# cnmoro/MiniVectorDB

Hardware: AMD Instinct MI355X
Metric: queries/sec + p50 latency, brute-force IP kNN, 10M×512 fp32, k=10 (higher is better)
Workload: dtype f32; 1 GPU; 10000000 x 512 fp32 corpus (10000000 rows resident per GPU), IP, k=10, nq=1 per step; rows_per_gpu=10000000, dim=512, k=10, nq=1, parallelism=row-sharded x1

## Files before the change

include/mvdb.h:

```cpp
#ifndef MVDB_H
#define MVDB_H

#include <stdint.h>

#ifdef __cplusplus
extern "C" {
#endif

#define MVDB_METRIC_IP 0
#define MVDB_METRIC_L2 1

#define MVDB_OK 0
#define MVDB_ERR_ARG 1
#define MVDB_ERR_HIP 2
#define MVDB_ERR_NODEVICE 3
#define MVDB_ERR_OOM 4

typedef struct mvdb_index mvdb_index;
typedef struct mvdb_encoder mvdb_encoder;


const char* mvdb_last_error(void);

int mvdb_abi_version(void);
// ... 14 lines not shown
int64_t mvdb_index_ntotal(const mvdb_index* idx);
int mvdb_index_dim(const mvdb_index* idx);
int mvdb_index_device(const mvdb_index* idx);

int64_t mvdb_index_shadow_rows(const mvdb_index* idx);

int64_t mvdb_index_code8_rows(const mvdb_index* idx);

int mvdb_index_code8_counters(const mvdb_index* idx, long long* fallbacks, long long* last_candidates, long long* calls);

int mvdb_code8_margin(int d, float qnorm, float qstep, float row_norm_bound, float* alpha, float* beta);

int mvdb_code8_pack(int d, const int8_t* codes, uint8_t* high, uint8_t* low);
int mvdb_code8_unpack(int d, const uint8_t* high, const uint8_t* low, int8_t* codes);

int mvdb_code8_front_pack(int d, const int8_t* codes, uint8_t* image);
int mvdb_code8_front_unpack(int d, const uint8_t* image, int8_t* codes);

int mvdb_code8_front_geometry(int d, int64_t n, int device, int* rows_per_batch, int* waves);

int mvdb_index_code8_front_counters(const mvdb_index* idx, long long* survivors, long long* calls, long long* suspensions, int* held);

int mvdb_index_code8_read_row(const mvdb_index* idx, int64_t row, uint8_t* high, uint8_t* low, uint8_t* front);

int mvdb_code8_scan_geometry(int d, int64_t n, int device, int* rows_per_batch, int* waves);

int mvdb_index_code8_refined(const mvdb_index* idx, long long* rows);

int mvdb_index_reserve(mvdb_index* idx, int64_t n);

int mvdb_index_add(mvdb_index* idx, const float* x_host, int64_t n, int normalize);

int mvdb_index_add_device(mvdb_index* idx, const float* x_dev, int64_t n, int normalize);

int mvdb_index_add_synthetic(mvdb_index* idx, int64_t n, uint64_t seed, int64_t first_row,
                             int normalize);

int mvdb_index_get_rows(const mvdb_index* idx, int64_t row0, int64_t n, float* out_host);

int mvdb_index_remove_rows(mvdb_index* idx, const int64_t* rows_host, int64_t m);

int mvdb_index_set_rows(mvdb_index* idx, const int64_t* rows_host, const float* x_host, int64_t m, int normalize);

int mvdb_index_set_rows_device(mvdb_index* idx, const int64_t* rows_host, const float* x_dev , int64_t m,
                               int normalize);

// ... 205 lines not shown
```

minivectordb_amd/_native.py:

```python
import ctypes
import os

import numpy as np

_HERE = os.path.dirname(os.path.abspath(__file__))
LIB_PATH = os.path.join(_HERE, "lib", "libmvdb.so")
LIB_PATH = os.environ.get("MVDB_LIBMVDB", LIB_PATH)

METRIC_IP = 0
METRIC_L2 = 1

ERR_ARG = 1
ERR_HIP = 2
ERR_NODEVICE = 3
ERR_OOM = 4

_lib = None

c_f32p = ctypes.POINTER(ctypes.c_float)
c_i64p = ctypes.POINTER(ctypes.c_int64)
c_i32p = ctypes.POINTER(ctypes.c_int32)
c_vp = ctypes.c_void_p


# ... 14 lines not shown

PROTOTYPES = {
    "mvdb_last_error": (ctypes.c_char_p, []),
    "mvdb_abi_version": (ctypes.c_int, []),
    "mvdb_device_count": (ctypes.c_int, [ctypes.POINTER(ctypes.c_int)]),
    "mvdb_index_create": (ctypes.c_int, [ctypes.c_int, ctypes.c_int, ctypes.c_int, ctypes.POINTER(c_vp)]),
    "mvdb_index_free": (ctypes.c_int, [c_vp]),
    "mvdb_index_reload_env": (ctypes.c_int, [c_vp]),
    "mvdb_index_set_option": (ctypes.c_int, [c_vp, ctypes.c_char_p, ctypes.c_longlong]),
    "mvdb_index_reset": (ctypes.c_int, [c_vp]),
    "mvdb_index_ntotal": (ctypes.c_int64, [c_vp]),
    "mvdb_index_shadow_rows": (ctypes.c_int64, [c_vp]),
    "mvdb_index_code8_rows": (ctypes.c_int64, [c_vp]),
    "mvdb_index_code8_counters": (ctypes.c_int, [c_vp, c_vp, c_vp, c_vp]),
    "mvdb_code8_margin": (ctypes.c_int, [ctypes.c_int, ctypes.c_float, ctypes.c_float, ctypes.c_float, c_vp, c_vp]),
    "mvdb_code8_pack": (ctypes.c_int, [ctypes.c_int, c_vp, c_vp, c_vp]),
    "mvdb_code8_unpack": (ctypes.c_int, [ctypes.c_int, c_vp, c_vp, c_vp]),
    "mvdb_index_code8_refined": (ctypes.c_int, [c_vp, c_vp]),
    "mvdb_code8_front_pack": (ctypes.c_int, [ctypes.c_int, c_vp, c_vp]),
    "mvdb_code8_front_unpack": (ctypes.c_int, [ctypes.c_int, c_vp, c_vp]),
    "mvdb_code8_front_geometry": (ctypes.c_int, [ctypes.c_int, ctypes.c_int64, ctypes.c_int, c_vp, c_vp]),
    "mvdb_index_code8_front_counters": (ctypes.c_int, [c_vp, c_vp, c_vp, c_vp, c_vp]),
    "mvdb_index_code8_read_row": (ctypes.c_int, [c_vp, ctypes.c_int64, c_vp, c_vp, c_vp]),
    "mvdb_code8_scan_geometry": (ctypes.c_int, [ctypes.c_int, ctypes.c_int64, ctypes.c_int, c_vp, c_vp]),
    "mvdb_index_dim": (ctypes.c_int, [c_vp]),
    "mvdb_index_device": (ctypes.c_int, [c_vp]),
    "mvdb_index_reserve": (ctypes.c_int, [c_vp, ctypes.c_int64]),
    "mvdb_index_add": (ctypes.c_int, [c_vp, c_vp, ctypes.c_int64, ctypes.c_int]),
    "mvdb_index_add_device": (ctypes.c_int, [c_vp, c_vp, ctypes.c_int64, ctypes.c_int]),
    "mvdb_index_add_synthetic": (ctypes.c_int, [c_vp, ctypes.c_int64, ctypes.c_uint64, ctypes.c_int64, ctypes.c_int]),
    "mvdb_index_get_rows": (ctypes.c_int, [c_vp, ctypes.c_int64, ctypes.c_int64, c_vp]),
    "mvdb_index_remove_rows": (ctypes.c_int, [c_vp, c_vp, ctypes.c_int64]),
    "mvdb_index_set_rows": (ctypes.c_int, [c_vp, c_vp, c_vp, ctypes.c_int64, ctypes.c_int]),
    "mvdb_index_set_rows_device": (ctypes.c_int, [c_vp, c_vp, c_vp, ctypes.c_int64, ctypes.c_int]),
    "mvdb_index_search": (ctypes.c_int, [c_vp, c_vp, ctypes.c_int, ctypes.c_int, ctypes.c_int, c_vp, c_vp]),
    "mvdb_index_search_device": (ctypes.c_int, [c_vp, c_vp, ctypes.c_int, ctypes.c_int, ctypes.c_int,
                                                ctypes.c_int64, c_vp, c_vp, c_vp]),
    "mvdb_index_search_subset": (ctypes.c_int, [c_vp, c_vp, ctypes.c_int, ctypes.c_int, ctypes.c_int, c_vp,
                                                ctypes.c_int64, c_vp, c_vp]),
    "mvdb_index_search_subset_device": (ctypes.c_int, [c_vp, c_vp, ctypes.c_int, ctypes.c_int, ctypes.c_int, c_vp,
                                                       ctypes.c_int64, ctypes.c_int, ctypes.c_int64, c_vp, c_vp, c_vp]),
    "mvdb_index_search_masked": (ctypes.c_int, [c_vp, c_vp, ctypes.c_int, ctypes.c_int, ctypes.c_int, c_vp, ctypes.c_int,
                                                c_vp, c_vp]),
    "mvdb_index_search_masked_device": (ctypes.c_int, [c_vp, c_vp, ctypes.c_int, ctypes.c_int, ctypes.c_int, c_vp,
                                                       ctypes.c_int, ctypes.c_int64, c_vp, c_vp, c_vp]),
    "mvdb_rowset_create": (ctypes.c_int, [c_vp, c_vp, ctypes.c_int64, ctypes.c_int, ctypes.POINTER(c_vp)]),
# ... 979 lines not shown

def code8_front_pack(codes):
    codes = np.ascontiguousarray(codes, dtype=np.int8)
    d = codes.shape[0]
    image = np.empty(max(d // 8 * 5, 1), np.uint8)
    check(lib().mvdb_code8_front_pack(int(d), codes.ctypes.data, image.ctypes.data))
    return image


def code8_front_unpack(image):
    image = np.ascontiguousarray(image, dtype=np.uint8)
    d = image.shape[0] // 5 * 8
    codes = np.empty(max(d, 1), np.int8)
    check(lib().mvdb_code8_front_unpack(int(d), image.ctypes.data, codes.ctypes.data))
    return codes


def code8_front_geometry(d, n, device=0):
    rb, waves = ctypes.c_int(0), ctypes.c_int(0)
    check(lib().mvdb_code8_front_geometry(int(d), int(n), int(device), ctypes.byref(rb), ctypes.byref(waves)))
    return int(rb.value), int(waves.value)


def code8_scan_geometry(d, n, device=0):
    rb, waves = ctypes.c_int(0), ctypes.c_int(0)
    check(lib().mvdb_code8_scan_geometry(int(d), int(n), int(device), ctypes.byref(rb), ctypes.byref(waves)))
    return int(rb.value), int(waves.value)
```

minivectordb_amd/csrc/code8_scan.hpp:

```cpp
#pragma once
#include "scan_kernels.hpp"

namespace mvdb {

typedef int i32x4 __attribute__((ext_vector_type(4)));

struct Code8Margin {
    float alpha, beta;
};
__host__ __device__ inline Code8Margin code8_margin(int d, float qnorm, float qstep, float row_norm_bound) {
    const double u = 5.9604644775390625e-08;
    const double qn = (double)qnorm, B = (double)row_norm_bound;
    const double dq = (double)qstep * sqrt((double)d) * 0.5 * 1.001 + qn * 4.0 * u;
    const double kap = 8.0 * u;
    const double gam = (d + 8) * u / (1.0 - (d + 8) * u);
    const double eta = 2.0 * (d + 16) * u;
    const double up = 1.0 + 9.5367431640625e-07;
    Code8Margin m;
    m.alpha = (float)((qn + dq) * (1.0 + kap) * up);
    m.beta = (float)(B * (dq + kap * (qn + dq) + (gam * (1.0 + eta) + eta) * qn) * up + 1e-30);
    return m;
}
__host__ __device__ inline int code8_qmax(int d) { return d <= 512 ? 32512 : 16256; }

// ... 27 lines not shown
#pragma unroll
    for (int i = 0; i < 4; ++i) c[i] |= lo[i];
}
inline void code8_pack_row(int d, const int8_t* codes, uint8_t* high, uint8_t* low) {
    for (int t = 0; t < d / 16; ++t) {
        uint32_t c[4], h[3], l;
        memcpy(c, codes + 16 * t, 16);
        code8_pack_chunk(c, h, l);
        memcpy(high + 12 * t, h, 12);
        memcpy(low + 4 * t, &l, 4);
    }
}
inline void code8_unpack_row(int d, const uint8_t* high, const uint8_t* low, int8_t* codes) {
    for (int t = 0; t < d / 16; ++t) {
        uint32_t c[4], h[3], l;
        memcpy(h, high + 12 * t, 12);
        memcpy(&l, low + 4 * t, 4);
        code8_unpack_chunk(h, l, c);
        memcpy(codes + 16 * t, c, 16);
    }
}

constexpr uint32_t kCode8FrontMask = 0xF8F8F8F8u;
__host__ __device__ inline bool code8_front_dim(int d) { return d > 0 && d % 32 == 0 && d <= 2048; }
__host__ __device__ inline int code8_front_stride(int d) { return d / 8 * 5; }
__host__ __device__ inline int code8_front_lanes(int d) {
    int g = 1;
    while (g * 32 < d) g *= 2;
    return g;
}
__host__ __device__ inline int code8_front_tile_rows(int d) { return 64 / code8_front_lanes(d); }
__host__ __device__ inline size_t code8_front_bytes(int64_t cap, int d) {
    const int64_t R = code8_front_tile_rows(d);
    return (size_t)((cap + R - 1) / R * R) * (size_t)code8_front_stride(d);
}
__host__ __device__ inline size_t code8_front_wide_offset(int64_t row, int d) {
    const int64_t R = code8_front_tile_rows(d);
    return (size_t)(row / R * R) * (size_t)code8_front_stride(d) + (size_t)(row % R) * (size_t)(d / 2);
}
__host__ __device__ inline size_t code8_front_narrow_offset(int64_t row, int d) {
    const int64_t R = code8_front_tile_rows(d);
    return (size_t)(row / R * R) * (size_t)code8_front_stride(d) + (size_t)R * (size_t)(d / 2) + (size_t)(row % R) * (size_t)(d / 8);
}

__host__ __device__ inline void code8_front_pack_chunk(const uint32_t (&c)[8], uint32_t (&f)[5]) {
    f[0] = (c[0] & kCode8FrontMask) | ((c[5] >> 5) & 0x07070707u);
    f[1] = (c[1] & kCode8FrontMask) | ((c[5] >> 3) & 0x03030303u) | ((c[7] >> 2) & 0x04040404u);
    f[2] = (c[2] & kCode8FrontMask) | ((c[6] >> 5) & 0x07070707u);
    f[3] = (c[3] & kCode8FrontMask) | ((c[6] >> 3) & 0x03030303u) | ((c[7] >> 1) & 0x04040404u);
    f[4] = (c[4] & kCode8FrontMask) | ((c[7] >> 5) & 0x07070707u);
}
__host__ __device__ inline void code8_front_unpack_chunk(const uint32_t (&f)[5], uint32_t (&c)[8]) {
#pragma unroll
    for (int i = 0; i < 5; ++i) c[i] = f[i] & kCode8FrontMask;
    c[5] = ((f[0] & 0x07070707u) << 5) | ((f[1] & 0x03030303u) << 3);
    c[6] = ((f[2] & 0x07070707u) << 5) | ((f[3] & 0x03030303u) << 3);
    c[7] = ((f[4] & 0x07070707u) << 5) | ((f[1] & 0x04040404u) << 2) | ((f[3] & 0x04040404u) << 1);
}
inline void code8_front_pack_row(int d, const int8_t* codes, uint8_t* image) {
    for (int t = 0; t < d / 32; ++t) {
        uint32_t c[8], f[5];
        memcpy(c, codes + 32 * t, 32);
        code8_front_pack_chunk(c, f);
        memcpy(image + 16 * t, f, 16);
        memcpy(image + d / 2 + 4 * t, &f[4], 4);
// ... 49 lines not shown
                    float cf = rintf(v[j] / a);
                    cf = fminf(fmaxf(cf, -127.f), 127.f);
                    const float e = fmaf(-a, cf, v[j]);
                    r2 = fmaf(e, e, r2);
                    word |= ((uint32_t)(uint8_t)(int8_t)(int)cf) << (8 * j);
                }
            }
            uint32_t chunk[4], h[3], l;
#pragma unroll
            for (int j = 0; j < 4; ++j) chunk[j] = (uint32_t)__shfl((int)word, (lane & ~3) + j);
            code8_pack_chunk(chunk, h, l);
            const int part = lane & 3;
            if (part < 3)
                hdst[3 * (c >> 2) + part] = part == 0 ? h[0] : part == 1 ? h[1] : h[2];
            else
                ldst[c >> 2] = l;
            if (front) {
                uint32_t oct[8], f[5];
#pragma unroll
                for (int j = 0; j < 8; ++j) oct[j] = (uint32_t)__shfl((int)word, (lane & ~7) + j);
                code8_front_pack_chunk(oct, f);
                const int fpart = lane & 7;
                if (fpart < 4)
                    reinterpret_cast<uint32_t*>(front + code8_front_wide_offset(front_row0 + row, d))[4 * (c >> 3) + fpart] =
                        fpart == 0 ? f[0] : fpart == 1 ? f[1] : fpart == 2 ? f[2] : f[3];
                else if (fpart == 4)
                    reinterpret_cast<uint32_t*>(front + code8_front_narrow_offset(front_row0 + row, d))[c >> 3] = f[4];
            }
        }
#pragma unroll
        for (int m = 32; m >= 1; m >>= 1) r2 += __shfl_xor(r2, m);
        if (lane == 0) {
            float r;
            if (anybad)
                r = INFINITY;
            else if (tiny)
                r = fmaf(mx, sqrtf((float)d) * 1.01f, 1e-44f);
            else
                r = sqrtf(r2 + (float)d * 2e-38f) * 1.001f;
            if (!(r < INFINITY)) r = INFINITY;
            ar[row] = make_float2(a, r);
        }
    }
}

constexpr int kCode8QueryThreads = 256;
constexpr int kCode8MaxDim = 1024;

struct Code8QueryShared {
    float nr[kCode8QueryThreads];
// ... 212 lines not shown

template <int G, int U, int M = 1>
__device__ __forceinline__ int code8_reduce(int (&T)[U], int t) {
    if constexpr (M < U) {
        constexpr int H = U / (2 * M);
        const bool hi = (t & M) != 0;
#pragma unroll
        for (int j = 0; j < H; ++j) {
            const int send = hi ? T[j] : T[j + H];
            const int keep = hi ? T[j + H] : T[j];
            T[j] = keep + lane_xor<M>(send);
        }
        return code8_reduce<G, U, M * 2>(T, t);
    } else if constexpr (M < G) {
        T[0] += lane_xor<M>(T[0]);
        return code8_reduce<G, U, M * 2>(T, t);
    } else {
        return T[0];
    }
}

typedef int i32x3 __attribute__((ext_vector_type(3), aligned(4)));

template <int G, int U, bool MASKED, int GF = 0, int UF = 0>
__global__ __launch_bounds__(kScanThreads) void code8_scan_kernel(Code8ScanArgs a) {
    constexpr int RPI = kWave / G;
    constexpr int RB = RPI * U;
    constexpr bool FRONT = GF > 0;
    static_assert(U >= 2 && U <= 8 && (U & (U - 1)) == 0 && U <= G, "code8_reduce halves U down to one value inside a row group");
    static_assert(!FRONT || (UF >= 2 && UF <= 8 && (UF & (UF - 1)) == 0 && UF <= GF && kWave % GF == 0), "the same, for the front form");
    const int lane = threadIdx.x & (kWave - 1);
    const int wave = __builtin_amdgcn_readfirstlane(threadIdx.x >> 6);
    const int t = lane % G;
    const int g = lane / G;
    const bool valid = !MASKED || t * 16 < a.d;

    i32x4 qh = {0, 0, 0, 0}, ql = {0, 0, 0, 0};
    if (valid) {
        qh = *reinterpret_cast<const i32x4*>(a.qhi + t * 16);
        ql = *reinterpret_cast<const i32x4*>(a.qlo + t * 16);
    }
    const float qstep = a.par[0], alpha = a.par[1], beta = a.par[2];
    float floor = 0.f;

    int p3 = 0, n3 = 0;
#pragma unroll
    for (int j = 0; j < 4; ++j) {
#pragma unroll
        for (int b = 0; b < 4; ++b) {
            const int Q = ((qh[j] << (24 - 8 * b)) >> 24) * 256 + ((ql[j] << (24 - 8 * b)) >> 24);
            p3 += Q > 0 ? Q : 0;
            n3 += Q < 0 ? -Q : 0;
        }
// ... 110 lines not shown
            const int src = __ffsll((long long)pass) - 1;
            pass &= pass - 1;
            const uint32_t v = (uint32_t)__builtin_amdgcn_readlane((int)r, src);
            const int w = __builtin_amdgcn_readlane(t6, src);
            if (lane == ns1) {
                srow = v;
                st6 = w;
            }
            if (++ns1 == kWave) refine();
        }
    };

    const int64_t nwaves_total = (int64_t)gridDim.x * kScanWaves;
    const int64_t gw = (int64_t)blockIdx.x * kScanWaves + wave;
    __shared__ uint64_t sh[(kScanWaves - 1) * kWave];
    __shared__ float sfloor;

    if constexpr (FRONT) {
        constexpr int RPF = kWave / GF;
        constexpr int RBF = RPF * UF;
        const int tf = lane % GF;
        const int gf = lane / GF;
        const bool validf = !MASKED || tf * 32 < a.d;
        i32x4 fh[2] = {{0, 0, 0, 0}, {0, 0, 0, 0}}, fl[2] = {{0, 0, 0, 0}, {0, 0, 0, 0}};
        if (validf) {
#pragma unroll
            for (int i = 0; i < 2; ++i) {
                fh[i] = *reinterpret_cast<const i32x4*>(a.qhi + tf * 32 + 16 * i);
                fl[i] = *reinterpret_cast<const i32x4*>(a.qlo + tf * 32 + 16 * i);
            }
        }
        int uef = 0;
#pragma unroll
        for (int m = 1, h = UF / 2; m < UF; m <<= 1, h >>= 1) uef += (tf & m) ? h : 0;
        const int erowf = uef * RPF + gf;
        const uint64_t elanesf = __ballot(tf < UF);

        if (blockIdx.x == 0 && threadIdx.x == 0) {
            const unsigned int calls = atomicAdd(a.front_calls, 1u);
            const unsigned long long sum = atomicAdd(a.front_survivors, 0ull);
            if (a.front_msum) {
                *a.front_msum = sum;
                *a.front_mcalls = calls;
            }
        }

        auto scores0 = [&](const i32x4 (&xw)[UF], const int (&xn)[UF], int (&T)[UF]) {
#pragma unroll
            for (int u = 0; u < UF; ++u) {
                const uint32_t f[5] = {(uint32_t)xw[u].x, (uint32_t)xw[u].y, (uint32_t)xw[u].z, (uint32_t)xw[u].w, (uint32_t)xn[u]};
                uint32_t c[8];
                code8_front_unpack_chunk(f, c);
                int hi = 0, lo = 0;
#pragma unroll
                for (int j = 0; j < 8; ++j) {
                    hi = __builtin_amdgcn_sdot4((int)c[j], fh[j >> 2][j & 3], hi, false);
                    lo = __builtin_amdgcn_sdot4((int)c[j], fl[j >> 2][j & 3], lo, false);
                }
                T[u] = hi * 256 + lo;
            }
        };
        uint32_t s0row = 0;
        int ns0 = 0;
        unsigned long long nfront = 0;
        auto gather0 = [&]() __attribute__((always_inline)) {
            nfront += (unsigned long long)ns0;
            for (int base = 0; base < ns0; base += RB) {
                i32x3 x[U];
#pragma unroll
                for (int u = 0; u < U; ++u) {
                    int e = base + u * RPI + g;
                    e = e < ns0 - 1 ? e : ns0 - 1;
                    const uint32_t row = (uint32_t)__shfl((int)s0row, e);
                    const i32x3* src = reinterpret_cast<const i32x3*>(a.high + (int64_t)row * a.hstride + t * 12);
                    if (MASKED)
                        x[u] = valid ? *src : i32x3{0, 0, 0};
                    else
                        x[u] = *src;
                }
                const int e = base + erow;
// ... 6 lines not shown
            }
            ns0 = 0;
        };
        auto stage0 = [&](int t5, float2 sr, uint64_t mine, int64_t r) __attribute__((always_inline)) {
            const int tl = (t5 > INT_MIN + n7 ? t5 : INT_MIN + n7) - n7;
            const float su = ((float)(t5 + p7) * qstep) * sr.x;
            const float sl = ((float)tl * qstep) * sr.x;
            float m = fmaf(alpha, sr.y, beta);
            m = fmaf(fmaxf(fabsf(su), fabsf(sl)) + m, 2.4e-7f, m);
            const float ub = su + m;
            uint64_t pass = __ballot(!(ub < floor)) & mine;
            while (pass) {
                const int src = __ffsll((long long)pass) - 1;
                pass &= pass - 1;
                const uint32_t v = (uint32_t)__builtin_amdgcn_readlane((int)r, src);
                if (lane == ns0) s0row = v;
                if (++ns0 == kWave) gather0();
            }
        };

        const int nch = a.d / 32;
        const int64_t tile_bytes = (int64_t)RPF * code8_front_stride(a.d);
        const int64_t batch_bytes = (int64_t)UF * tile_bytes;
        const int wide_off = gf * 16 * nch + tf * 16;
        const int narrow_off = RPF * 16 * nch + gf * 4 * nch + tf * 4;
        const int64_t nfull = a.n / RBF;
        auto load0 = [&](i32x4 (&xw)[UF], int (&xn)[UF], float2& sr, int64_t b) {
            const uint8_t* base = a.front + b * batch_bytes;
#pragma unroll
            for (int u = 0; u < UF; ++u) {
                const i32x4* ws = reinterpret_cast<const i32x4*>(base + u * tile_bytes + wide_off);
                const int* ns = reinterpret_cast<const int*>(base + u * tile_bytes + narrow_off);
                if (MASKED) {
                    xw[u] = validf ? __builtin_nontemporal_load(ws) : i32x4{0, 0, 0, 0};
                    xn[u] = validf ? __builtin_nontemporal_load(ns) : 0;
                } else {
                    xw[u] = __builtin_nontemporal_load(ws);
                    xn[u] = __builtin_nontemporal_load(ns);
                }
            }
            sr = a.ar[b * RBF + erowf];
        };
        int64_t b = gw;
        const bool head = b < nfull;
        i32x4 xw0[UF];
        int xn0[UF];
        float2 sr0 = make_float2(0.f, 0.f);
        if (head) load0(xw0, xn0, sr0, b);
        floor = __uint_as_float((uint32_t)__builtin_amdgcn_readfirstlane(
            (int)__float_as_uint(code8_lists_floor(a.lists, a.nlists, a.k, sh, &sfloor, kScanWaves))));
        if (blockIdx.x == 0 && threadIdx.x == 0) *a.floor = floor;
        if (head) {
            int T[UF];
            scores0(xw0, xn0, T);
            stage0(code8_reduce<GF, UF>(T, tf), sr0, elanesf, b * RBF + erowf);
            b += nwaves_total;
        }
        for (; b < nfull; b += nwaves_total) {
            i32x4 xw[UF];
            int xn[UF];
            float2 sr;
            load0(xw, xn, sr, b);
            int T[UF];
            scores0(xw, xn, T);
            stage0(code8_reduce<GF, UF>(T, tf), sr, elanesf, b * RBF + erowf);
        }
        if (nfull * RBF < a.n && nfull % nwaves_total == gw) {
            const int64_t last = a.n - 1;
            const int64_t last_tile = last / RPF;
            i32x4 xw[UF];
            int xn[UF];
#pragma unroll
            for (int u = 0; u < UF; ++u) {
                int64_t tile = nfull * UF + u;
                tile = tile < last_tile ? tile : last_tile;
                const uint8_t* base = a.front + tile * tile_bytes;
                const i32x4* ws = reinterpret_cast<const i32x4*>(base + wide_off);
                const int* ns = reinterpret_cast<const int*>(base + narrow_off);
                if (MASKED) {
                    xw[u] = validf ? __builtin_nontemporal_load(ws) : i32x4{0, 0, 0, 0};
                    xn[u] = validf ? __builtin_nontemporal_load(ns) : 0;
                } else {
                    xw[u] = __builtin_nontemporal_load(ws);
                    xn[u] = __builtin_nontemporal_load(ns);
                }
            }
            const int64_t r = nfull * RBF + erowf;
            const float2 sr = a.ar[r < last ? r : last];
            int T[UF];
            scores0(xw, xn, T);
            stage0(code8_reduce<GF, UF>(T, tf), sr, __ballot(tf < UF && r < a.n), r);
        }
        if (ns0) gather0();
        if (ns1) refine();
        if (nfront && lane == 0) atomicAdd(a.front_survivors, nfront);
        if (nrefined && lane == 0) atomicAdd(a.survivors, nrefined);
        if (nst) flush();
        return;
    }

    const int64_t nfull = a.n / RB;
    const int64_t batch_bytes = (int64_t)RB * a.hstride;
    const int64_t group_bytes = (int64_t)RPI * a.hstride;
    const int lane_off = g * a.hstride + t * 12;

    auto load = [&](i32x3 (&x)[U], float2& sr, int64_t b) {
        const uint8_t* base = a.high + b * batch_bytes + lane_off;
#pragma unroll
// ... 386 lines not shown
```

minivectordb_amd/csrc/mvdb.hip:

```cpp
#include <algorithm>
#include <cmath>
#include <cstdlib>
#include <atomic>
#include <functional>
#include <map>
#include <tuple>
#include <vector>
#include <shared_mutex>

#include "common.hpp"
#include "index_state.hpp"
#include "scan_kernels.hpp"
#include "grouped_scan.hpp"
#include "range_scan.hpp"
#include "join_scan.hpp"
#include "mmr_select.hpp"
#include "distinct_select.hpp"
#include "maxsim_scan.hpp"
#include "assign_scan.hpp"
#include "code8_scan.hpp"
#include "scan_mfma_kernels.hpp"
#include "select_kernels.hpp"
#include "half_scan.hpp"
#include "util_kernels.hpp"
// ... 1820 lines not shown
    rows = idx->n + n_new;
    return 0;
}

bool code8_route_ok(const mvdb_index* idx, int nq, int k, const int64_t* rows_dev, const uint64_t* mask_dev, int64_t n) {
    if (nq != 1 || !idx->kn.code8_single_query || idx->kn.shadow_single_query) return false;
    if (idx->metric != MVDB_METRIC_IP || rows_dev || mask_dev || k > kMaxFusedK) return false;
    if (n != idx->n || n < kCode8MinRows || !code8_dim(idx->d) || idx->ld != idx->d) return false;
    if (!(idx->row_norm_bound > 0.f) || !(idx->row_norm_bound < 1.0e30f) || idx->code.failed) return false;
    return true;
}

template <int G_, int U_, bool MASKED_, int SCAN_U_, int SCAN_BLOCKS_, int FRONT_G_, int FRONT_U_, int FRONT_BLOCKS_, bool FRONT_DEFAULT_>
struct Code8Shape {
    static constexpr bool FRONT_DEFAULT = FRONT_DEFAULT_;
    static constexpr int G = G_, U = U_, SCAN_U = SCAN_U_, SCAN_BLOCKS = SCAN_BLOCKS_;
    static constexpr int FRONT_G = FRONT_G_, FRONT_U = FRONT_U_, FRONT_BLOCKS = FRONT_BLOCKS_;
    static constexpr bool MASKED = MASKED_;
};
template <typename Launch>
int with_code8_shape(int d, Launch launch) {
    switch (d) {
        case 384: return launch(Code8Shape<32, 8, true, 8, 4, 16, 8, 2, true>{});
        case 512: return launch(Code8Shape<32, 4, false, 8, 2, 16, 4, 2, true>{});
        case 1024: return launch(Code8Shape<64, 4, false, 8, 2, 32, 4, 2, false>{});
        default: return fail(MVDB_ERR_ARG, "internal: no int8 prefilter kernel for d = %d", d);
    }
}
template <typename Launch>
int with_code8_exact_shape(int d4, Launch launch) {
    return with_scan_shape(d4, [&](auto shape) {
        if constexpr (code8_shape(decltype(shape)::G, decltype(shape)::C)) return launch(shape);
        else return fail(MVDB_ERR_ARG, "internal: no int8 prefilter kernel for rows of %d 16-byte chunks", d4);
    });
}

bool code8_front_wanted(int option, int d) {
    if (option == 0 || !code8_dim(d) || !code8_front_dim(d)) return false;
    bool dflt = false;
    (void)with_code8_shape(d, [&](auto cs) {
        dflt = decltype(cs)::FRONT_DEFAULT;
        return 0;
    });
    return option >= 2 || dflt;
}

template <int G, int U, bool MASKED, int BLOCKS, int GF = 0, int UF = 0>
int code8_scan_blocks(int64_t n, int device) {
    void (*kern)(Code8ScanArgs) = code8_scan_kernel<G, U, MASKED, GF, UF>;
    int per_cu = std::min(cached_occupancy((const void*)kern, kScanThreads, 0, 4), BLOCKS);
    if (kn().scan_blocks_per_cu > 0) per_cu = kn().scan_blocks_per_cu;
    return scan_grid(n, GF > 0 ? (kWave / GF) * UF : (kWave / G) * U, per_cu, device);
}
template <int G, int U, bool MASKED, int BLOCKS, int GF = 0, int UF = 0>
int launch_code8_scan(const Code8ScanArgs& a, int device, hipStream_t stream) {
    void (*kern)(Code8ScanArgs) = code8_scan_kernel<G, U, MASKED, GF, UF>;
    const int nblocks = code8_scan_blocks<G, U, MASKED, BLOCKS, GF, UF>(a.n, device);
    if constexpr (GF > 0)
        return profiled_launch("ip_scan", stream, [&](hipEvent_t done) { launch_kernel(kern, dim3(nblocks), dim3(kScanThreads), 0, stream, done, a); },
                               "code8_scan_kernel<%d, %d, %s, %d, %d>", G, U, MASKED ? "true" : "false", GF, UF);
    else
        return profiled_launch("ip_scan", stream, [&](hipEvent_t done) { launch_kernel(kern, dim3(nblocks), dim3(kScanThreads), 0, stream, done, a); },
                               "code8_scan_kernel<%d, %d, %s>", G, U, MASKED ? "true" : "false");
}
constexpr double kCode8FrontShare = 0.12;
bool code8_front_serves(const mvdb_index* idx) {
    if (!idx->code.F5.p || !code8_front_wanted(idx->kn.code8_front_plane, idx->d)) return false;
    if (idx->kn.code8_front_plane >= 2) return idx->kn.code8_front_plane == 2;
    const volatile unsigned long long* sum = idx->c8_ctr.mirror<unsigned long long>();
    return !idx->c8_front.suspended_mean(sum ? sum + 2 : nullptr, idx->c8_ctr.mirror() ? idx->c8_ctr.mirror() + 6 : nullptr,
                                         kCode8FrontShare * (double)idx->n);
}

template <int G, int U, bool MASKED>
int launch_code8_seed(const Code8SeedArgs& a, int device, hipStream_t stream, int* nlists) {
    void (*kern)(Code8SeedArgs) = code8_seed_kernel<G, U, MASKED>;
    int threads = kn().code8_seed_threads;
    if (threads != 256 && threads != 512 && threads != 1024) threads = kCode8SeedThreads;
    constexpr int64_t nbatches = kCode8Seed / ((kWave / G) * U);
    const int64_t want = (nbatches + threads / kWave - 1) / (threads / kWave);
    int64_t blocks = kn().code8_seed_blocks > 0 ? kn().code8_seed_blocks : device_cus(device);
    blocks = std::max<int64_t>(1, std::min<int64_t>(std::min<int64_t>(blocks, want), scan_grid_upper_bound(device)));
    *nlists = (int)blocks;
    return profiled_launch("ip_scan_code8_seed", stream, [&](hipEvent_t done) { launch_kernel(kern, dim3((unsigned)blocks), dim3(threads), 0, stream, done, a); },
                           "code8_seed_kernel<%d, %d, %s>", G, U, MASKED ? "true" : "false");
}

template <int G, int C, int U, bool MASKED>
int launch_code8_rescore(const Code8RescoreArgs& a, int device, hipStream_t stream) {
    void (*kern)(Code8RescoreArgs) = code8_rescore_kernel<G, C, U, MASKED>;
    const int64_t want = (a.cap + a.rows_per_block - 1) / a.rows_per_block;
    const int64_t blocks = std::max<int64_t>(1, std::min<int64_t>(want, (int64_t)device_cus(device) * 4));
    return profiled_launch("ip_scan_code8_rescore", stream, [&](hipEvent_t done) { launch_kernel(kern, dim3((unsigned)blocks), dim3(kScanThreads), 0, stream, done, a); },
                           "code8_rescore_kernel<%d, %d, %d, %s>", G, C, U, MASKED ? "true" : "false");
// ... 56 lines not shown
    c.n = idx->n;
    c.d = d;
    c.hstride = code8_high_stride(d);
    c.qhi = qhi;
    c.qlo = qlo;
    c.par = par;
    c.lists = ws->cand.p;
    c.nlists = seed_lists;
    c.k = k;
    c.floor = floor;
    c.cand = cand;
    c.cap = cap;
    c.counter = counter;
    c.survivors = reinterpret_cast<unsigned long long*>(idx->c8_ctr.dev() + 2);
    c.front = idx->code.F5.p;
    c.front_survivors = reinterpret_cast<unsigned long long*>(idx->c8_ctr.dev() + 4);
    c.front_calls = idx->c8_ctr.dev() + 6;
    c.front_msum = idx->c8_ctr.mirror<unsigned long long>() + 2;
    c.front_mcalls = idx->c8_ctr.mirror() + 6;
    const bool front = code8_front_serves(idx);
    MVDB_TRY(with_code8_shape(d, [&](auto cs) {
        using K = decltype(cs);
        if (!front) return launch_code8_scan<K::G, K::SCAN_U, K::MASKED, K::SCAN_BLOCKS>(c, idx->device, s);
        const int fu = kn().code8_front_u == 4 || kn().code8_front_u == 8 ? kn().code8_front_u : K::FRONT_U;
        if (fu == 4) return launch_code8_scan<K::G, K::SCAN_U, K::MASKED, K::FRONT_BLOCKS, K::FRONT_G, 4>(c, idx->device, s);
        return launch_code8_scan<K::G, K::SCAN_U, K::MASKED, K::FRONT_BLOCKS, K::FRONT_G, 8>(c, idx->device, s);
    }));
    Code8RescoreArgs r;
    r.X = a0.X;
    r.ld = a0.ld;
    r.d4 = a0.d4;
    r.q = a0.q;
    r.normalize_q = a0.normalize_q;
    r.k = k;
    r.cand = cand;
    r.counter = counter;
    r.cap = cap;
    r.par = par;
    r.rows_per_block = kn().code8_rescore_rows > 0 ? kn().code8_rescore_rows : kCode8RescoreRows;
    r.lists = ws->cand.p;
    r.active = active;
    r.gate = gate;
    r.ctr_dev = idx->c8_ctr.dev();
    r.stats = idx->c8_ctr.mirror();
    MVDB_TRY(with_code8_exact_shape(a0.d4, [&](auto shape) {
        using S = decltype(shape);
        return launch_code8_rescore<S::G, S::C, rescore_u(S::G, S::C), false>(r, idx->device, s);
    }));
    ScanArgs a = a0;
// ... 319 lines not shown
        std::lock_guard<std::mutex> lk(idx->shadow_mu);
        *held = idx->code.F5.p ? 1 : 0;
    }
    if (!idx->c8_ctr.dev()) return 0;
    DeviceGuard dg(idx->device);
    unsigned int w[3] = {0, 0, 0};
    MVDB_HIP(hipMemcpy(w, idx->c8_ctr.dev() + 4, sizeof(w), hipMemcpyDeviceToHost));
    if (survivors) *survivors = (long long)((unsigned long long)w[0] | ((unsigned long long)w[1] << 32));
    if (calls) *calls = (long long)w[2];
    return 0;
}
int mvdb_index_code8_read_row(const mvdb_index* idx, int64_t row, uint8_t* high, uint8_t* low, uint8_t* front) {
    if (!idx) return fail(MVDB_ERR_ARG, "index is NULL");
    std::shared_lock<std::shared_mutex> lk(idx->mu);
    std::lock_guard<std::mutex> sk(idx->shadow_mu);
    const Code8Store& c = idx->code;
    if (!c.C8.p || row < 0 || row >= c.rows) return fail(MVDB_ERR_ARG, "mvdb_index_code8_read_row: row %lld is not in the code", (long long)row);
    if (front && !c.F5.p) return fail(MVDB_ERR_ARG, "mvdb_index_code8_read_row: the code holds no front plane");
    DeviceGuard dg(idx->device);
    const int d = idx->d;
    if (high) MVDB_HIP(hipMemcpy(high, c.C8.p + row * code8_high_stride(d), code8_high_stride(d), hipMemcpyDeviceToHost));
    if (low) MVDB_HIP(hipMemcpy(low, c.low(d) + row * code8_low_stride(d), code8_low_stride(d), hipMemcpyDeviceToHost));
    if (front) {
        MVDB_HIP(hipMemcpy(front, c.F5.p + code8_front_wide_offset(row, d), d / 2, hipMemcpyDeviceToHost));
        MVDB_HIP(hipMemcpy(front + d / 2, c.F5.p + code8_front_narrow_offset(row, d), d / 8, hipMemcpyDeviceToHost));
    }
    return 0;
}
int mvdb_code8_margin(int d, float qnorm, float qstep, float row_norm_bound, float* alpha, float* beta) {
    if (d <= 0 || !alpha || !beta) return fail(MVDB_ERR_ARG, "mvdb_code8_margin: bad arguments");
    const Code8Margin m = code8_margin(d, qnorm, qstep, row_norm_bound);
    *alpha = m.alpha;
    *beta = m.beta;
    return 0;
}
int mvdb_index_dim(const mvdb_index* idx) { return idx ? idx->d : -1; }
int mvdb_index_device(const mvdb_index* idx) { return idx ? idx->device : -1; }

int mvdb_index_reserve(mvdb_index* idx, int64_t n) {
    if (!idx) return fail(MVDB_ERR_ARG, "index is NULL");
    if (n < 0) return fail(MVDB_ERR_ARG, "negative row count");
    std::unique_lock<std::shared_mutex> lk(idx->mu);
    DeviceGuard dg(idx->device);
    if (n <= idx->cap) return 0;
    MVDB_TRY(quiesce(idx));
    return grow(idx, n, true);
}

static int note_row_norms(mvdb_index* idx, const float* dst, int64_t n, int normalize, const int64_t* list_dev = nullptr) {
// ... 2282 lines not shown
```

Measured before the change: 1836 queries/s.

## Interleave the d=512 front plane into four chunk slabs per lane

For d=512 the packed 5-bit front plane is re-laid out so that each lane handles four 32-dim chunks. The wide parts go into per-chunk slabs, and one 16-byte narrow load covers all four chunks. Front lanes drop from 16 to 4, and the unroll defaults change to match, so each lane issues larger contiguous loads and each wave covers more rows per tile. The front-plane suspension threshold is also lowered for this layout. This changes the on-device format, so the packer, the row reader and a new offset query are updated to keep them consistent.

```diff
diff --git a/include/mvdb.h b/include/mvdb.h
--- a/include/mvdb.h
+++ b/include/mvdb.h
@@ -60,6 +60,8 @@
 int mvdb_index_code8_front_counters(const mvdb_index* idx, long long* survivors, long long* calls, long long* suspensions, int* held);
 
 int mvdb_index_code8_read_row(const mvdb_index* idx, int64_t row, uint8_t* high, uint8_t* low, uint8_t* front);
+
+int mvdb_code8_front_offset(int d, int64_t row, int chunk, int64_t* wide, int64_t* narrow);
 
 int mvdb_code8_scan_geometry(int d, int64_t n, int device, int* rows_per_batch, int* waves);
 
diff --git a/minivectordb_amd/_native.py b/minivectordb_amd/_native.py
--- a/minivectordb_amd/_native.py
+++ b/minivectordb_amd/_native.py
@@ -60,6 +60,7 @@
     "mvdb_code8_front_geometry": (ctypes.c_int, [ctypes.c_int, ctypes.c_int64, ctypes.c_int, c_vp, c_vp]),
     "mvdb_index_code8_front_counters": (ctypes.c_int, [c_vp, c_vp, c_vp, c_vp, c_vp]),
     "mvdb_index_code8_read_row": (ctypes.c_int, [c_vp, ctypes.c_int64, c_vp, c_vp, c_vp]),
+    "mvdb_code8_front_offset": (ctypes.c_int, [ctypes.c_int, ctypes.c_int64, ctypes.c_int, c_vp, c_vp]),
     "mvdb_code8_scan_geometry": (ctypes.c_int, [ctypes.c_int, ctypes.c_int64, ctypes.c_int, c_vp, c_vp]),
     "mvdb_index_dim": (ctypes.c_int, [c_vp]),
     "mvdb_index_device": (ctypes.c_int, [c_vp]),
@@ -1085,6 +1086,12 @@
     return int(rb.value), int(waves.value)
 
 
+def code8_front_offset(d, row, chunk):
+    wide, narrow = ctypes.c_int64(0), ctypes.c_int64(0)
+    check(lib().mvdb_code8_front_offset(int(d), int(row), int(chunk), ctypes.byref(wide), ctypes.byref(narrow)))
+    return int(wide.value), int(narrow.value)
+
+
 def code8_scan_geometry(d, n, device=0):
     rb, waves = ctypes.c_int(0), ctypes.c_int(0)
     check(lib().mvdb_code8_scan_geometry(int(d), int(n), int(device), ctypes.byref(rb), ctypes.byref(waves)))
diff --git a/minivectordb_amd/csrc/code8_scan.hpp b/minivectordb_amd/csrc/code8_scan.hpp
--- a/minivectordb_amd/csrc/code8_scan.hpp
+++ b/minivectordb_amd/csrc/code8_scan.hpp
@@ -73,25 +73,44 @@
 }
 
 constexpr uint32_t kCode8FrontMask = 0xF8F8F8F8u;
+#ifdef MVDB_CODE8_ABLATE
+constexpr int kCode8QuadDim = 0;
+#else
+constexpr int kCode8QuadDim = 512;
+#endif
+constexpr int kCode8QuadChunks = 4;
 __host__ __device__ inline bool code8_front_dim(int d) { return d > 0 && d % 32 == 0 && d <= 2048; }
 __host__ __device__ inline int code8_front_stride(int d) { return d / 8 * 5; }
-__host__ __device__ inline int code8_front_lanes(int d) {
+__host__ __device__ constexpr int code8_front_lanes(int d) {
+    if (d == kCode8QuadDim) return d / (32 * kCode8QuadChunks);
     int g = 1;
     while (g * 32 < d) g *= 2;
     return g;
 }
+__host__ __device__ constexpr bool code8_front_quad(int d) { return code8_front_lanes(d) * 32 * kCode8QuadChunks == d; }
 __host__ __device__ inline int code8_front_tile_rows(int d) { return 64 / code8_front_lanes(d); }
 __host__ __device__ inline size_t code8_front_bytes(int64_t cap, int d) {
     const int64_t R = code8_front_tile_rows(d);
     return (size_t)((cap + R - 1) / R * R) * (size_t)code8_front_stride(d);
 }
-__host__ __device__ inline size_t code8_front_wide_offset(int64_t row, int d) {
+__host__ __device__ inline size_t code8_front_wide_offset(int64_t row, int chunk, int d) {
     const int64_t R = code8_front_tile_rows(d);
-    return (size_t)(row / R * R) * (size_t)code8_front_stride(d) + (size_t)(row % R) * (size_t)(d / 2);
-}
-__host__ __device__ inline size_t code8_front_narrow_offset(int64_t row, int d) {
+    const size_t tile = (size_t)(row / R * R) * (size_t)code8_front_stride(d);
+    if (code8_front_quad(d)) {
+        const int L = code8_front_lanes(d);
+        return tile + (size_t)(chunk % kCode8QuadChunks) * (size_t)(R * L * 16) + (size_t)((row % R) * L + chunk / kCode8QuadChunks) * 16;
+    }
+    return tile + (size_t)(row % R) * (size_t)(d / 2) + (size_t)chunk * 16;
+}
+__host__ __device__ inline size_t code8_front_narrow_offset(int64_t row, int chunk, int d) {
     const int64_t R = code8_front_tile_rows(d);
-    return (size_t)(row / R * R) * (size_t)code8_front_stride(d) + (size_t)R * (size_t)(d / 2) + (size_t)(row % R) * (size_t)(d / 8);
+    const size_t tile = (size_t)(row / R * R) * (size_t)code8_front_stride(d);
+    if (code8_front_quad(d)) {
+        const int L = code8_front_lanes(d);
+        return tile + (size_t)kCode8QuadChunks * (size_t)(R * L * 16) + (size_t)((row % R) * L + chunk / kCode8QuadChunks) * 16 +
+               (size_t)(chunk % kCode8QuadChunks) * 4;
+    }
+    return tile + (size_t)R * (size_t)(d / 2) + (size_t)(row % R) * (size_t)(d / 8) + (size_t)chunk * 4;
 }
 
 __host__ __device__ inline void code8_front_pack_chunk(const uint32_t (&c)[8], uint32_t (&f)[5]) {
@@ -187,10 +206,10 @@
                 code8_front_pack_chunk(oct, f);
                 const int fpart = lane & 7;
                 if (fpart < 4)
-                    reinterpret_cast<uint32_t*>(front + code8_front_wide_offset(front_row0 + row, d))[4 * (c >> 3) + fpart] =
+                    reinterpret_cast<uint32_t*>(front + code8_front_wide_offset(front_row0 + row, c >> 3, d))[fpart] =
                         fpart == 0 ? f[0] : fpart == 1 ? f[1] : fpart == 2 ? f[2] : f[3];
                 else if (fpart == 4)
-                    reinterpret_cast<uint32_t*>(front + code8_front_narrow_offset(front_row0 + row, d))[c >> 3] = f[4];
+                    *reinterpret_cast<uint32_t*>(front + code8_front_narrow_offset(front_row0 + row, c >> 3, d)) = f[4];
             }
         }
 #pragma unroll
@@ -449,13 +468,25 @@
 
 typedef int i32x3 __attribute__((ext_vector_type(3), aligned(4)));
 
+template <bool QUAD>
+struct Code8Narrow {
+    typedef int type;
+    static __device__ __forceinline__ int part(int v, int) { return v; }
+};
+template <>
+struct Code8Narrow<true> {
+    typedef i32x4 type;
+    static __device__ __forceinline__ int part(const i32x4& v, int s) { return v[s]; }
+};
+
 template <int G, int U, bool MASKED, int GF = 0, int UF = 0>
 __global__ __launch_bounds__(kScanThreads) void code8_scan_kernel(Code8ScanArgs a) {
     constexpr int RPI = kWave / G;
     constexpr int RB = RPI * U;
     constexpr bool FRONT = GF > 0;
     static_assert(U >= 2 && U <= 8 && (U & (U - 1)) == 0 && U <= G, "code8_reduce halves U down to one value inside a row group");
-    static_assert(!FRONT || (UF >= 2 && UF <= 8 && (UF & (UF - 1)) == 0 && UF <= GF && kWave % GF == 0), "the same, for the front form");
+    constexpr bool QUAD = FRONT && !MASKED && GF * 32 * kCode8QuadChunks == G * 16;
+    static_assert(!FRONT || (UF >= (QUAD ? 1 : 2) && UF <= 8 && (UF & (UF - 1)) == 0 && UF <= GF && kWave % GF == 0), "the same, for the front form");
     const int lane = threadIdx.x & (kWave - 1);
     const int wave = __builtin_amdgcn_readfirstlane(threadIdx.x >> 6);
     const int t = lane % G;
@@ -612,12 +643,19 @@
         const int tf = lane % GF;
         const int gf = lane / GF;
         const bool validf = !MASKED || tf * 32 < a.d;
-        i32x4 fh[2] = {{0, 0, 0, 0}, {0, 0, 0, 0}}, fl[2] = {{0, 0, 0, 0}, {0, 0, 0, 0}};
-        if (validf) {
+        constexpr int NC = QUAD ? kCode8QuadChunks : 1;
+        typedef typename Code8Narrow<QUAD>::type narrow_t;
+        i32x4 fh[NC][2], fl[NC][2];
+#pragma unroll
+        for (int s = 0; s < NC; ++s) {
 #pragma unroll
             for (int i = 0; i < 2; ++i) {
-                fh[i] = *reinterpret_cast<const i32x4*>(a.qhi + tf * 32 + 16 * i);
-                fl[i] = *reinterpret_cast<const i32x4*>(a.qlo + tf * 32 + 16 * i);
+                fh[s][i] = i32x4{0, 0, 0, 0};
+                fl[s][i] = i32x4{0, 0, 0, 0};
+                if (validf) {
+                    fh[s][i] = *reinterpret_cast<const i32x4*>(a.qhi + (tf * NC + s) * 32 + 16 * i);
+                    fl[s][i] = *reinterpret_cast<const i32x4*>(a.qlo + (tf * NC + s) * 32 + 16 * i);
+                }
             }
         }
         int uef = 0;
@@ -635,17 +673,21 @@
             }
         }
 
-        auto scores0 = [&](const i32x4 (&xw)[UF], const int (&xn)[UF], int (&T)[UF]) {
+        auto scores0 = [&](const i32x4 (&xw)[UF][NC], const narrow_t (&xn)[UF], int (&T)[UF]) {
 #pragma unroll
             for (int u = 0; u < UF; ++u) {
-                const uint32_t f[5] = {(uint32_t)xw[u].x, (uint32_t)xw[u].y, (uint32_t)xw[u].z, (uint32_t)xw[u].w, (uint32_t)xn[u]};
-                uint32_t c[8];
-                code8_front_unpack_chunk(f, c);
                 int hi = 0, lo = 0;
 #pragma unroll
-                for (int j = 0; j < 8; ++j) {
-                    hi = __builtin_amdgcn_sdot4((int)c[j], fh[j >> 2][j & 3], hi, false);
-                    lo = __builtin_amdgcn_sdot4((int)c[j], fl[j >> 2][j & 3], lo, false);
+                for (int s = 0; s < NC; ++s) {
+                    const uint32_t f[5] = {(uint32_t)xw[u][s].x, (uint32_t)xw[u][s].y, (uint32_t)xw[u][s].z, (uint32_t)xw[u][s].w,
+                                           (uint32_t)Code8Narrow<QUAD>::part(xn[u], s)};
+                    uint32_t c[8];
+                    code8_front_unpack_chunk(f, c);
+#pragma unroll
+                    for (int j = 0; j < 8; ++j) {
+                        hi = __builtin_amdgcn_sdot4((int)c[j], fh[s][j >> 2][j & 3], hi, false);
+                        lo = __builtin_amdgcn_sdot4((int)c[j], fl[s][j >> 2][j & 3], lo, false);
+                    }
                 }
                 T[u] = hi * 256 + lo;
             }
@@ -698,29 +740,40 @@
         const int nch = a.d / 32;
         const int64_t tile_bytes = (int64_t)RPF * code8_front_stride(a.d);
         const int64_t batch_bytes = (int64_t)UF * tile_bytes;
-        const int wide_off = gf * 16 * nch + tf * 16;
-        const int narrow_off = RPF * 16 * nch + gf * 4 * nch + tf * 4;
+        constexpr int slab = QUAD ? kWave * 16 : 0;
+        const int wide_off = QUAD ? lane * 16 : gf * 16 * nch + tf * 16;
+        const int narrow_off = QUAD ? NC * slab + lane * 16 : RPF * 16 * nch + gf * 4 * nch + tf * 4;
         const int64_t nfull = a.n / RBF;
-        auto load0 = [&](i32x4 (&xw)[UF], int (&xn)[UF], float2& sr, int64_t b) {
+        auto load_tile = [&](const uint8_t* tile, i32x4 (&w)[NC], narrow_t& nr) __attribute__((always_inline)) {
+            const narrow_t* ns = reinterpret_cast<const narrow_t*>(tile + narrow_off);
+#pragma unroll
+            for (int s = 0; s < NC; ++s) {
+                const i32x4* ws = reinterpret_cast<const i32x4*>(tile + s * slab + wide_off);
+                if (MASKED)
+                    w[s] = validf ? __builtin_nontemporal_load(ws) : i32x4{0, 0, 0, 0};
+                else
+                    w[s] = __builtin_nontemporal_load(ws);
+            }
+#ifdef MVDB_CODE8_ABLATE
+            nr = narrow_t{};
+            (void)ns;
+#else
+            if (MASKED)
+                nr = validf ? __builtin_nontemporal_load(ns) : narrow_t{};
+            else
+                nr = __builtin_nontemporal_load(ns);
+#endif
+        };
+        auto load0 = [&](i32x4 (&xw)[UF][NC], narrow_t (&xn)[UF], float2& sr, int64_t b) {
             const uint8_t* base = a.front + b * batch_bytes;
 #pragma unroll
-            for (int u = 0; u < UF; ++u) {
-                const i32x4* ws = reinterpret_cast<const i32x4*>(base + u * tile_bytes + wide_off);
-                const int* ns = reinterpret_cast<const int*>(base + u * tile_bytes + narrow_off);
-                if (MASKED) {
-                    xw[u] = validf ? __builtin_nontemporal_load(ws) : i32x4{0, 0, 0, 0};
-                    xn[u] = validf ? __builtin_nontemporal_load(ns) : 0;
-                } else {
-                    xw[u] = __builtin_nontemporal_load(ws);
-                    xn[u] = __builtin_nontemporal_load(ns);
-                }
-            }
+            for (int u = 0; u < UF; ++u) load_tile(base + u * tile_bytes, xw[u], xn[u]);
             sr = a.ar[b * RBF + erowf];
         };
         int64_t b = gw;
         const bool head = b < nfull;
-        i32x4 xw0[UF];
-        int xn0[UF];
+        i32x4 xw0[UF][NC];
+        narrow_t xn0[UF];
         float2 sr0 = make_float2(0.f, 0.f);
         if (head) load0(xw0, xn0, sr0, b);
         floor = __uint_as_float((uint32_t)__builtin_amdgcn_readfirstlane(
@@ -733,8 +786,8 @@
             b += nwaves_total;
         }
         for (; b < nfull; b += nwaves_total) {
-            i32x4 xw[UF];
-            int xn[UF];
+            i32x4 xw[UF][NC];
+            narrow_t xn[UF];
             float2 sr;
             load0(xw, xn, sr, b);
             int T[UF];
@@ -744,22 +797,13 @@
         if (nfull * RBF < a.n && nfull % nwaves_total == gw) {
             const int64_t last = a.n - 1;
             const int64_t last_tile = last / RPF;
-            i32x4 xw[UF];
-            int xn[UF];
+            i32x4 xw[UF][NC];
+            narrow_t xn[UF];
 #pragma unroll
             for (int u = 0; u < UF; ++u) {
                 int64_t tile = nfull * UF + u;
                 tile = tile < last_tile ? tile : last_tile;
-                const uint8_t* base = a.front + tile * tile_bytes;
-                const i32x4* ws = reinterpret_cast<const i32x4*>(base + wide_off);
-                const int* ns = reinterpret_cast<const int*>(base + narrow_off);
-                if (MASKED) {
-                    xw[u] = validf ? __builtin_nontemporal_load(ws) : i32x4{0, 0, 0, 0};
-                    xn[u] = validf ? __builtin_nontemporal_load(ns) : 0;
-                } else {
-                    xw[u] = __builtin_nontemporal_load(ws);
-                    xn[u] = __builtin_nontemporal_load(ns);
-                }
+                load_tile(a.front + tile * tile_bytes, xw[u], xn[u]);
             }
             const int64_t r = nfull * RBF + erowf;
             const float2 sr = a.ar[r < last ? r : last];
diff --git a/minivectordb_amd/csrc/mvdb.hip b/minivectordb_amd/csrc/mvdb.hip
--- a/minivectordb_amd/csrc/mvdb.hip
+++ b/minivectordb_amd/csrc/mvdb.hip
@@ -1866,7 +1866,7 @@
 int with_code8_shape(int d, Launch launch) {
     switch (d) {
         case 384: return launch(Code8Shape<32, 8, true, 8, 4, 16, 8, 2, true>{});
-        case 512: return launch(Code8Shape<32, 4, false, 8, 2, 16, 4, 2, true>{});
+        case 512: return launch(Code8Shape<32, 4, false, 8, 2, code8_front_lanes(512), code8_front_quad(512) ? 2 : 4, code8_front_quad(512) ? 1 : 2, true>{});
         case 1024: return launch(Code8Shape<64, 4, false, 8, 2, 32, 4, 2, false>{});
         default: return fail(MVDB_ERR_ARG, "internal: no int8 prefilter kernel for d = %d", d);
     }
@@ -1907,13 +1907,13 @@
         return profiled_launch("ip_scan", stream, [&](hipEvent_t done) { launch_kernel(kern, dim3(nblocks), dim3(kScanThreads), 0, stream, done, a); },
                                "code8_scan_kernel<%d, %d, %s>", G, U, MASKED ? "true" : "false");
 }
-constexpr double kCode8FrontShare = 0.12;
+constexpr double kCode8FrontShare = 0.12, kCode8FrontShareQuad = 0.08;
 bool code8_front_serves(const mvdb_index* idx) {
     if (!idx->code.F5.p || !code8_front_wanted(idx->kn.code8_front_plane, idx->d)) return false;
     if (idx->kn.code8_front_plane >= 2) return idx->kn.code8_front_plane == 2;
     const volatile unsigned long long* sum = idx->c8_ctr.mirror<unsigned long long>();
     return !idx->c8_front.suspended_mean(sum ? sum + 2 : nullptr, idx->c8_ctr.mirror() ? idx->c8_ctr.mirror() + 6 : nullptr,
-                                         kCode8FrontShare * (double)idx->n);
+                                         (code8_front_quad(idx->d) ? kCode8FrontShareQuad : kCode8FrontShare) * (double)idx->n);
 }
 
 template <int G, int U, bool MASKED>
@@ -2016,9 +2016,17 @@
     MVDB_TRY(with_code8_shape(d, [&](auto cs) {
         using K = decltype(cs);
         if (!front) return launch_code8_scan<K::G, K::SCAN_U, K::MASKED, K::SCAN_BLOCKS>(c, idx->device, s);
-        const int fu = kn().code8_front_u == 4 || kn().code8_front_u == 8 ? kn().code8_front_u : K::FRONT_U;
-        if (fu == 4) return launch_code8_scan<K::G, K::SCAN_U, K::MASKED, K::FRONT_BLOCKS, K::FRONT_G, 4>(c, idx->device, s);
-        return launch_code8_scan<K::G, K::SCAN_U, K::MASKED, K::FRONT_BLOCKS, K::FRONT_G, 8>(c, idx->device, s);
+        const int hook = kn().code8_front_u;
+        if constexpr (code8_front_quad(K::G * 16) && !K::MASKED) {
+            const int fu = hook == 1 || hook == 2 || hook == 4 ? hook : K::FRONT_U;
+            if (fu == 1) return launch_code8_scan<K::G, K::SCAN_U, K::MASKED, K::FRONT_BLOCKS, K::FRONT_G, 1>(c, idx->device, s);
+            if (fu == 2) return launch_code8_scan<K::G, K::SCAN_U, K::MASKED, K::FRONT_BLOCKS, K::FRONT_G, 2>(c, idx->device, s);
+            return launch_code8_scan<K::G, K::SCAN_U, K::MASKED, K::FRONT_BLOCKS, K::FRONT_G, 4>(c, idx->device, s);
+        } else {
+            const int fu = hook == 4 || hook == 8 ? hook : K::FRONT_U;
+            if (fu == 4) return launch_code8_scan<K::G, K::SCAN_U, K::MASKED, K::FRONT_BLOCKS, K::FRONT_G, 4>(c, idx->device, s);
+            return launch_code8_scan<K::G, K::SCAN_U, K::MASKED, K::FRONT_BLOCKS, K::FRONT_G, 8>(c, idx->device, s);
+        }
     }));
     Code8RescoreArgs r;
     r.X = a0.X;
@@ -2384,9 +2392,23 @@
     if (high) MVDB_HIP(hipMemcpy(high, c.C8.p + row * code8_high_stride(d), code8_high_stride(d), hipMemcpyDeviceToHost));
     if (low) MVDB_HIP(hipMemcpy(low, c.low(d) + row * code8_low_stride(d), code8_low_stride(d), hipMemcpyDeviceToHost));
     if (front) {
-        MVDB_HIP(hipMemcpy(front, c.F5.p + code8_front_wide_offset(row, d), d / 2, hipMemcpyDeviceToHost));
-        MVDB_HIP(hipMemcpy(front + d / 2, c.F5.p + code8_front_narrow_offset(row, d), d / 8, hipMemcpyDeviceToHost));
-    }
+        const int64_t R = code8_front_tile_rows(d);
+        const size_t tile_bytes = (size_t)R * (size_t)code8_front_stride(d);
+        const size_t tile_at = (size_t)(row / R * R) * (size_t)code8_front_stride(d);
+        std::vector<uint8_t> tile(tile_bytes);
+        MVDB_HIP(hipMemcpy(tile.data(), c.F5.p + tile_at, tile_bytes, hipMemcpyDeviceToHost));
+        for (int t = 0; t < d / 32; ++t) {
+            memcpy(front + 16 * t, tile.data() + (code8_front_wide_offset(row, t, d) - tile_at), 16);
+            memcpy(front + d / 2 + 4 * t, tile.data() + (code8_front_narrow_offset(row, t, d) - tile_at), 4);
+        }
+    }
+    return 0;
+}
+int mvdb_code8_front_offset(int d, int64_t row, int chunk, int64_t* wide, int64_t* narrow) {
+    if (!code8_front_dim(d) || row < 0 || chunk < 0 || chunk >= d / 32 || !wide || !narrow)
+        return fail(MVDB_ERR_ARG, "mvdb_code8_front_offset: bad arguments (d a multiple of 32, at most 2048; chunk in [0, d / 32))");
+    *wide = (int64_t)code8_front_wide_offset(row, chunk, d);
+    *narrow = (int64_t)code8_front_narrow_offset(row, chunk, d);
     return 0;
 }
 int mvdb_code8_margin(int d, float qnorm, float qstep, float row_norm_bound, float* alpha, float* beta) {
```

Measured after the change: 1901 queries/s, median of 6. 3.6% higher.
